# ramanathanlab/molecular_dynamics_neural_operator

Measured on AMD Instinct MI355X. Metric: rolled-out MD frames/sec, higher is better.
Workload: dtype f32

## Files before the change

molecular_dynamics_neural_operator_amd/csrc/moment.hip:

```cpp
#include <type_traits>

#include "kernels.h"
#include "mfma_f32.h"
#include "moment_layout.h"
#include "split_mma.h"

namespace mdno {
namespace {

typedef float f32x4 __attribute__((ext_vector_type(4)));


__global__ __launch_bounds__(256) void w3_moment_kernel(const float* __restrict__ w3, const float* __restrict__ b3, int k,
                                                        float* __restrict__ w3r) {
    const long long id = (long long)blockIdx.x * 256 + threadIdx.x;
    const long long total = (long long)(64 * k + 64) * 64;
    if (id >= total) return;
    const int kl = (int)(id & 31), o = (int)((id >> 5) & 63);
    const long long kappa = (id >> 11) * 32 + kl;
    if (kappa >= (long long)64 * k) {
        w3r[id] = b3[(kappa - (long long)64 * k) * 64 + o];
        return;
    }
    const int i = (int)(kappa / k), c = (int)(kappa - (long long)i * k);
    w3r[id] = w3[((size_t)i * 64 + o) * k + c];
}

__global__ __launch_bounds__(256) void w3_colmax_kernel(const float* __restrict__ w3r, long long ntiles, int* __restrict__ colmax_bits) {
    __shared__ int red[4][64];
    const int o = threadIdx.x & 63, sub = threadIdx.x >> 6;
    float m = 0.f;
    for (long long t = (long long)blockIdx.x * 4 + sub; t < ntiles; t += (long long)gridDim.x * 4) {
        const float4* row = reinterpret_cast<const float4*>(w3r + (t * 64 + o) * 32);
#pragma unroll
        for (int j = 0; j < 8; ++j) {
            const float4 v = row[j];
            const float a = fabsf(v.x), b = fabsf(v.y), c = fabsf(v.z), d = fabsf(v.w);
            m = (a > m || a != a) ? a : m; m = (b > m || b != b) ? b : m;
            m = (c > m || c != c) ? c : m; m = (d > m || d != d) ? d : m;
        }
    }
    red[sub][o] = __builtin_bit_cast(int, m);
    __syncthreads();
    if (sub == 0) {
        int v = red[0][o];
        for (int u = 1; u < 4; ++u) v = red[u][o] > v ? red[u][o] : v;
        atomicMax(colmax_bits + o, v);
    }
}

__global__ __launch_bounds__(256) void w3_planes_f16_kernel(const float* __restrict__ w3r, long long total,
                                                            const int* __restrict__ colmax_bits, _Float16* __restrict__ w3h,
                                                            float* __restrict__ colinv) {
    const long long id = (long long)blockIdx.x * 256 + threadIdx.x;
    if (id < 64) colinv[id] = 1.f / f16_row_scale(__builtin_bit_cast(float, colmax_bits[id]));
    if (id >= total) return;
    const int kl = (int)(id & 31), o = (int)((id >> 5) & 63);
    const long long tile = id >> 11;
    const float v = w3r[id] * f16_row_scale(__builtin_bit_cast(float, colmax_bits[o]));
    const _Float16 h = (_Float16)v;
    w3h[(tile * 2 + 0) * 2048 + o * 32 + kl] = h;
    w3h[(tile * 2 + 1) * 2048 + o * 32 + kl] = (_Float16)(v - (float)h);
}

template <int CH>
__global__ __launch_bounds__(CH) void degree_order_kernel(const int* __restrict__ row_ptr, int num_rows,
                                                          int* __restrict__ order) {
    __shared__ __attribute__((aligned(16))) int key[CH];
    const int base = blockIdx.x * CH, t = threadIdx.x;
    const int cnt = num_rows - base < CH ? num_rows - base : CH;
    int dg = t < cnt ? row_ptr[base + t + 1] - row_ptr[base + t] : 0;
    dg = dg < (1 << 20) ? dg : (1 << 20);
    const int mine = t < cnt ? dg * CH + (CH - 1 - t) : -1;
    key[t] = mine;
    __syncthreads();
    if (t >= cnt) return;
    int rank = 0;
#pragma unroll 4
    for (int u = 0; u < CH; u += 4) {
        const int4 k4 = *reinterpret_cast<const int4*>(&key[u]);
        rank += (k4.x > mine) + (k4.y > mine) + (k4.z > mine) + (k4.w > mine);
    }
    order[base + rank] = t;
}

constexpr int MO_EDGES = 16;
constexpr size_t kMomentCachedBytes = (size_t)64 << 20;
constexpr int MO_HROW = MO_CQ * 2 + 64;
constexpr int MO_XROW = 64 * 2 + 64;
constexpr int MO_HPLANE = MO_EDGES * MO_HROW, MO_XPLANE = MO_EDGES * MO_XROW;
constexpr int MO_LDS = 3 * MO_HPLANE + 3 * MO_XPLANE;

__device__ __forceinline__ int f32_exponent(float p2) { return (int)((__builtin_bit_cast(unsigned, p2) >> 23) & 0xffu) - 127; }

__device__ __forceinline__ float wave_max(float v) {
#pragma unroll
    for (int off = 32; off > 0; off >>= 1) v = fmaxf(v, __shfl_xor(v, off, 64));
    return v;
}

__device__ __forceinline__ void moment_s0(const int* __restrict__ row_ptr, const int* __restrict__ src,
                                          const float* __restrict__ x, float* __restrict__ S, int K, int t, int tl,
                                          float* __restrict__ rowmax_slot, float scale) {
    __shared__ float4 sred[16][16];
    const int tid = threadIdx.x;
    const int beg = row_ptr[t], end = row_ptr[t + 1];
    const int es = tid >> 4, q = tid & 15;
    float4 s0 = make_float4(0.f, 0.f, 0.f, 0.f);
    for (int p = beg + es; p < end; p += 64) {
        int sj[4];
        bool on[4];
#pragma unroll
        for (int u = 0; u < 4; ++u) {
            on[u] = p + 16 * u < end;
            sj[u] = on[u] ? src[p + 16 * u] : 0;
        }
        float4 g[4];
#pragma unroll
        for (int u = 0; u < 4; ++u)
            g[u] = on[u] ? *reinterpret_cast<const float4*>(x + (size_t)sj[u] * 64 + 4 * q) : make_float4(0.f, 0.f, 0.f, 0.f);
#pragma unroll
        for (int u = 0; u < 4; ++u) { s0.x += g[u].x; s0.y += g[u].y; s0.z += g[u].z; s0.w += g[u].w; }
    }
    sred[es][q] = s0;
    __syncthreads();
    float4 s0r = make_float4(0.f, 0.f, 0.f, 0.f);
    if (es == 0) {
        float4 a = make_float4(0.f, 0.f, 0.f, 0.f);
#pragma unroll
        for (int c = 0; c < 16; ++c) { const float4 v = sred[c][q]; a.x += v.x; a.y += v.y; a.z += v.z; a.w += v.w; }
        a.x *= scale; a.y *= scale; a.z *= scale; a.w *= scale;
        s0r = a;
        const int i = 4 * q;
        float* d = S + ((size_t)(tl >> 7) * moment_nkt(K) + (size_t)64 * K / 32 + (i >> 5)) * 4096 + (tl & 127) * 32 + (i & 31);
        *reinterpret_cast<float4*>(d) = a;
    }
    if (rowmax_slot != nullptr && tid < 64) {
        float m = es == 0 ? fmaxf(fmaxf(fabsf(s0r.x), fabsf(s0r.y)), fmaxf(fabsf(s0r.z), fabsf(s0r.w))) : 0.f;
        m = wave_max(m);
        if (tid == 0) *rowmax_slot = m;
    }
}

constexpr int MOMENT_CNT_K1_RERUN = 0;
constexpr int MOMENT_CNT_X_PLAIN = 1;
constexpr int MO_F16_PRE_H_EXP = 5;
constexpr float MO_F16_PRE_H = 32.f, MO_F16_H_LIM = F16_MAX / 32.f, MO_F16_H_MIN = 0.25f / 32.f;

template <bool F16>
__global__ __launch_bounds__(256, 3) void moment_kernel(const float* __restrict__ Hm,
                                                        const int* __restrict__ row_ptr, const int* __restrict__ src,
                                                        const int* __restrict__ order, float* __restrict__ S, int K,
                                                        int row0, int cnt, const float* __restrict__ x, int cache_e,
                                                        float* __restrict__ rowmax, const float* __restrict__ xm,
                                                        int* __restrict__ counters) {
    __shared__ __attribute__((aligned(16))) unsigned char lds[MO_LDS];
    __shared__ float wg_red[12];
    const int nq = (K + MO_CQ - 1) / MO_CQ + 1;
    const int xcd = blockIdx.x & 7, rr = blockIdx.x >> 3;
    const int cq = rr % nq, ti = (rr / nq) * 8 + xcd;
    if (ti >= cnt) return;
    const int tl = order[row0 + ti];
    const int t = row0 + tl;
    const int beg = row_ptr[t], end = row_ptr[t + 1];
    const int tid = threadIdx.x, lane = tid & 63;
    const int wave = __builtin_amdgcn_readfirstlane(tid >> 6);
    const int nkt = K >> 5;
    float xsc = 1.f, hsc = 1.f;
    bool x_plain = false;
    if constexpr (F16) {
        float m = 0.f;
        for (int e = beg + tid; e < end; e += 256) m = fmaxf(m, xm[src[e]]);
        m = wave_max(m);
        if (lane == 0) wg_red[wave] = m;
        __syncthreads();
        m = fmaxf(fmaxf(wg_red[0], wg_red[1]), fmaxf(wg_red[2], wg_red[3]));
        x_plain = !(m >= 0x1p-100f && m < 0x1p100f);
        xsc = x_plain ? 1.f : __builtin_bit_cast(float, __builtin_amdgcn_readfirstlane(__builtin_bit_cast(int, f16_row_scale(m))));
        hsc = x_plain ? 1.f : MO_F16_PRE_H;
        __syncthreads();
        if (cq == 0 && tid == 0) {
            rowmax[(size_t)tl * (nq + 1) + nq] = x_plain ? 0.f : (float)(f32_exponent(xsc) + MO_F16_PRE_H_EXP);
            if (x_plain) atomicAdd(counters + MOMENT_CNT_X_PLAIN, 1);
        }
    }
    if (cq == nq - 1) {
        moment_s0(row_ptr, src, x, S, K, t, tl, rowmax ? rowmax + (size_t)tl * (nq + 1) + cq : nullptr, xsc * hsc);
        return;
    }
    const int er = tid >> 4, cc = tid & 15;
    const int xe = tid >> 4, xs = tid & 15;
    auto h_ptr = [&](int e, int u) {
        const int c = cq * MO_CQ + u * 64 + cc * 4;
        return Hm + ((size_t)(e >> 7) * nkt + (c >> 5)) * 4096 + (e & 127) * 32 + (c & 31);
    };
    float4 rh[4], rx;
    int sidx = 0;
#define MO_NT(DST, P)                                                                               \
    {                                                                                               \
        const f32x4 t_ = __builtin_nontemporal_load(reinterpret_cast<const f32x4*>(P));             \
        DST = make_float4(t_.x, t_.y, t_.z, t_.w);                                                  \
    }
    auto load_stage = [&](int e0) {
        const int e = e0 + er;
        if (e0 + MO_EDGES <= cache_e) {
#pragma unroll
            for (int u = 0; u < 4; ++u) {
                rh[u] = make_float4(0.f, 0.f, 0.f, 0.f);
                if (e < end && cq * MO_CQ + u * 64 < K) rh[u] = *reinterpret_cast<const float4*>(h_ptr(e, u));
            }
        } else {
#pragma unroll
            for (int u = 0; u < 4; ++u) {
                rh[u] = make_float4(0.f, 0.f, 0.f, 0.f);
                if (e < end && cq * MO_CQ + u * 64 < K) MO_NT(rh[u], h_ptr(e, u))
            }
        }
        rx = make_float4(0.f, 0.f, 0.f, 0.f);
        if (e0 + xe < end) rx = *reinterpret_cast<const float4*>(x + (size_t)sidx * 64 + 4 * xs);
    };
    const int gq = lane >> 4, qq = (lane >> 2) & 3, pp = lane & 3;
    const int frow = 8 * (gq >> 1) + qq, fcol = 16 * (gq & 1) + 4 * pp;
    const unsigned char* hb = lds + frow * MO_HROW + (wave * 64 + fcol) * 2;
    const unsigned char* xb = lds + 3 * MO_HPLANE + frow * MO_XROW + fcol * 2;
    auto tr_frag = [&](const unsigned char* p_, int row_bytes) {
        typedef short s16x4 __attribute__((ext_vector_type(4)));
        typedef __attribute__((address_space(3))) s16x4 lds_s16x4;
        const s16x4 lo = __builtin_amdgcn_ds_read_tr16_b64_v4i16((lds_s16x4*)(p_));
        const s16x4 hi = __builtin_amdgcn_ds_read_tr16_b64_v4i16((lds_s16x4*)(p_ + 4 * row_bytes));
        return __builtin_shufflevector(lo, hi, 0, 1, 2, 3, 4, 5, 6, 7);
    };
    f32x16 acc[2][2];
    const int stages = (end - beg + MO_EDGES - 1) / MO_EDGES;
    const bool wave_live = cq * MO_CQ + wave * 64 < K;
    float hmax = 0.f;
    auto max4 = [](const float4 v) { return fmaxf(fmaxf(fabsf(v.x), fabsf(v.y)), fmaxf(fabsf(v.z), fabsf(v.w))); };
    auto pre = [](const float4 v, float sc) { return make_float4(v.x * sc, v.y * sc, v.z * sc, v.w * sc); };
    auto wg_max2 = [&](float a, float b, float& ra, float& rb) {
        a = wave_max(a); b = wave_max(b);
        if (lane == 0) { wg_red[wave] = a; wg_red[4 + wave] = b; }
        __syncthreads();
        ra = fmaxf(fmaxf(wg_red[0], wg_red[1]), fmaxf(wg_red[2], wg_red[3]));
        rb = fmaxf(fmaxf(wg_red[4], wg_red[5]), fmaxf(wg_red[6], wg_red[7]));
    };

    auto run = [&](auto half_tag) {
        constexpr bool HALF = decltype(half_tag)::value;
        auto store_stage = [&]() {
            if constexpr (HALF) {
#pragma unroll
                for (int u = 0; u < 4; ++u) {
                    hmax = fmaxf(hmax, max4(rh[u]));
                    split2_store4(pre(rh[u], hsc), lds + er * MO_HROW + (u * 64 + cc * 4) * 2, MO_HPLANE);
                }
                split2_store4(pre(rx, xsc), lds + 3 * MO_HPLANE + xe * MO_XROW + xs * 8, MO_XPLANE);
            } else if constexpr (F16) {
#pragma unroll
                for (int u = 0; u < 4; ++u)
                    split_store4(pre(rh[u], hsc), lds + er * MO_HROW + (u * 64 + cc * 4) * 2, MO_HPLANE);
                split_store4(pre(rx, xsc), lds + 3 * MO_HPLANE + xe * MO_XROW + xs * 8, MO_XPLANE);
            } else {
#pragma unroll
                for (int u = 0; u < 4; ++u)
                    split_store4(rh[u], lds + er * MO_HROW + (u * 64 + cc * 4) * 2, MO_HPLANE);
                split_store4(rx, lds + 3 * MO_HPLANE + xe * MO_XROW + xs * 8, MO_XPLANE);
            }
        };
#pragma unroll
        for (int i = 0; i < 2; ++i)
#pragma unroll
            for (int j = 0; j < 2; ++j)
#pragma unroll
                for (int e = 0; e < 16; ++e) acc[i][j][e] = 0.f;
        if (stages == 0) return;
        sidx = 0;
        if (beg + xe < end) sidx = src[beg + xe];
        load_stage(beg);
        if (beg + MO_EDGES + xe < end) sidx = src[beg + MO_EDGES + xe];
        store_stage();
        __syncthreads();
        for (int st = 0; st < stages; ++st) {
            const int e_next = beg + (st + 1) * MO_EDGES;
            if (st + 1 < stages) {
                load_stage(e_next);
                if (e_next + MO_EDGES + xe < end) sidx = src[e_next + MO_EDGES + xe];
            }
            __builtin_amdgcn_sched_barrier(0);
            if (wave_live) {
                if constexpr (HALF) {
                    f16x8 a[2][2], b[2];
#pragma unroll
                    for (int ih = 0; ih < 2; ++ih)
#pragma unroll
                        for (int p = 0; p < 2; ++p)
                            a[ih][p] = __builtin_bit_cast(f16x8, tr_frag(xb + p * MO_XPLANE + ih * 64, MO_XROW));
#pragma unroll
                    for (int cb = 0; cb < 2; ++cb) {
#pragma unroll
                        for (int p = 0; p < 2; ++p) b[p] = __builtin_bit_cast(f16x8, tr_frag(hb + p * MO_HPLANE + cb * 64, MO_HROW));
                        mma3_f16(a[0], b, acc[0][cb]);
                        mma3_f16(a[1], b, acc[1][cb]);
                    }
                } else {
                    bf16x8 a[2][3], b[3];
#pragma unroll
                    for (int ih = 0; ih < 2; ++ih)
#pragma unroll
                        for (int p = 0; p < 3; ++p)
                            a[ih][p] = __builtin_bit_cast(bf16x8, tr_frag(xb + p * MO_XPLANE + ih * 64, MO_XROW));
#pragma unroll
                    for (int cb = 0; cb < 2; ++cb) {
#pragma unroll
                        for (int p = 0; p < 3; ++p) b[p] = __builtin_bit_cast(bf16x8, tr_frag(hb + p * MO_HPLANE + cb * 64, MO_HROW));
                        mma6_bf16(a[0], b, acc[0][cb]);
                        mma6_bf16(a[1], b, acc[1][cb]);
                    }
                }
            }
            if (st + 1 < stages) {
                __syncthreads();
                store_stage();
                __syncthreads();
            }
        }
    };
    if constexpr (F16) {
        run(std::true_type{});
        float mh, d;
        wg_max2(hmax, 0.f, mh, d);
        if (stages != 0 && (x_plain || !(mh < MO_F16_H_LIM && mh >= MO_F16_H_MIN))) {
            if (tid == 0) atomicAdd(counters + MOMENT_CNT_K1_RERUN, 1);
            __syncthreads();
            run(std::false_type{});
        }
    } else {
        run(std::false_type{});
    }
#undef MO_NT
    float smax = 0.f;
    if (wave_live) {
        const int l31 = lane & 31, h = lane >> 5;
        float* Sb = S + (size_t)(tl >> 7) * moment_nkt(K) * 4096 + (tl & 127) * 32 + l31;
#pragma unroll
        for (int ih = 0; ih < 2; ++ih)
#pragma unroll
            for (int cb = 0; cb < 2; ++cb) {
                const int c0 = cq * MO_CQ + wave * 64 + cb * 32;
#pragma unroll
                for (int e = 0; e < 16; ++e) {
                    const int i = mfma32_row(e, h, ih * 32);
                    const size_t kt = ((size_t)i * K + c0) >> 5;
                    const float v = acc[ih][cb][e];
                    Sb[kt * 4096] = v;
                    smax = fmaxf(smax, fabsf(v));
                }
            }
    }
    if (rowmax != nullptr) {
        __syncthreads();
        float m, d;
        wg_max2(smax, 0.f, m, d);
        if (tid == 0) rowmax[(size_t)tl * (nq + 1) + cq] = m;
    }
}

constexpr int MF_HLD = MO_CQ + 32, MF_XLD = 64 + 32;

__global__ __launch_bounds__(256) void moment_f32_kernel(const float* __restrict__ Hm, const int* __restrict__ row_ptr,
                                                         const int* __restrict__ src, const int* __restrict__ order,
                                                         float* __restrict__ S, int K, int row0, int cnt,
                                                         const float* __restrict__ x) {
    __shared__ __attribute__((aligned(16))) float hs[MO_EDGES * MF_HLD];
    __shared__ __attribute__((aligned(16))) float xs_[MO_EDGES * MF_XLD];
    const int nq = (K + MO_CQ - 1) / MO_CQ + 1;
    const int xcd = blockIdx.x & 7, rr = blockIdx.x >> 3;
    const int cq = rr % nq, ti = (rr / nq) * 8 + xcd;
    if (ti >= cnt) return;
    const int tl = order[row0 + ti];
    const int t = row0 + tl;
    if (cq == nq - 1) {
        moment_s0(row_ptr, src, x, S, K, t, tl, nullptr, 1.f);
        return;
    }
    const int beg = row_ptr[t], end = row_ptr[t + 1];
    const int tid = threadIdx.x, lane = tid & 63;
    const int wave = __builtin_amdgcn_readfirstlane(tid >> 6);
    const int er = tid >> 4, cc = tid & 15;
    const int l31 = lane & 31, h = lane >> 5;
    const bool wave_live = cq * MO_CQ + wave * 64 < K;
    f32x16 acc[2][2];
#pragma unroll
    for (int i = 0; i < 2; ++i)
#pragma unroll
        for (int j = 0; j < 2; ++j)
#pragma unroll
            for (int e = 0; e < 16; ++e) acc[i][j][e] = 0.f;
    for (int e0 = beg; e0 < end; e0 += MO_EDGES) {
        const int e = e0 + er;
        float4 rh[4], rx = make_float4(0.f, 0.f, 0.f, 0.f);
#pragma unroll
        for (int u = 0; u < 4; ++u) {
            rh[u] = make_float4(0.f, 0.f, 0.f, 0.f);
            const int c = cq * MO_CQ + u * 64 + cc * 4;
            if (e < end && c < K)
                rh[u] = *reinterpret_cast<const float4*>(Hm + ((size_t)(e >> 7) * (K >> 5) + (c >> 5)) * 4096 + (e & 127) * 32 + (c & 31));
        }
        if (e < end) rx = *reinterpret_cast<const float4*>(x + (size_t)src[e] * 64 + 4 * cc);
        __syncthreads();
#pragma unroll
        for (int u = 0; u < 4; ++u) *reinterpret_cast<float4*>(&hs[er * MF_HLD + u * 64 + cc * 4]) = rh[u];
        *reinterpret_cast<float4*>(&xs_[er * MF_XLD + cc * 4]) = rx;
        __syncthreads();
        if (wave_live) {
#pragma unroll
            for (int ks = 0; ks < MO_EDGES / 2; ++ks) {
                const float a0 = xs_[(2 * ks + h) * MF_XLD + l31], a1 = xs_[(2 * ks + h) * MF_XLD + 32 + l31];
                const float b0 = hs[(2 * ks + h) * MF_HLD + wave * 64 + l31], b1 = hs[(2 * ks + h) * MF_HLD + wave * 64 + 32 + l31];
                acc[0][0] = __builtin_amdgcn_mfma_f32_32x32x2f32(a0, b0, acc[0][0], 0, 0, 0);
                acc[0][1] = __builtin_amdgcn_mfma_f32_32x32x2f32(a0, b1, acc[0][1], 0, 0, 0);
                acc[1][0] = __builtin_amdgcn_mfma_f32_32x32x2f32(a1, b0, acc[1][0], 0, 0, 0);
                acc[1][1] = __builtin_amdgcn_mfma_f32_32x32x2f32(a1, b1, acc[1][1], 0, 0, 0);
            }
        }
    }
    if (!wave_live) return;
    float* Sb = S + (size_t)(tl >> 7) * moment_nkt(K) * 4096 + (tl & 127) * 32 + l31;
#pragma unroll
    for (int ih = 0; ih < 2; ++ih)
#pragma unroll
        for (int cb = 0; cb < 2; ++cb) {
            const int c0 = cq * MO_CQ + wave * 64 + cb * 32;
#pragma unroll
            for (int e = 0; e < 16; ++e) {
                const int i = mfma32_row(e, h, ih * 32);
                const size_t kt = ((size_t)i * K + c0) >> 5;
                Sb[kt * 4096] = acc[ih][cb][e];
            }
        }
}

constexpr int PJ_SLICES = 128;
constexpr int PJ_B_PLANE = 64 * 64;

template <int PJ_ROWS>
__global__ __launch_bounds__(PJ_ROWS * 2) void project_kernel(const float* __restrict__ S, const float* __restrict__ w3r,
                                                         float* __restrict__ part, int K, int cnt, int row0,
                                                         long long part_stride) {
    constexpr int PJ_A_PLANE = PJ_ROWS * 64, PJ_B_BASE = 3 * PJ_A_PLANE, NT = PJ_ROWS / 128;
    constexpr int RQ = PJ_ROWS / 4;
    __shared__ __attribute__((aligned(16))) unsigned char lds[3 * PJ_A_PLANE + 3 * PJ_B_PLANE];
    const int ngrp = gridDim.x / PJ_SLICES;
    const int xcd = blockIdx.x & 7, rr = blockIdx.x >> 3;
    const int rg = rr % ngrp, slice = (rr / ngrp) * 8 + xcd;
    const int tid = threadIdx.x, lane = tid & 63;
    const int wave = __builtin_amdgcn_readfirstlane(tid >> 6);
    const int l31 = lane & 31, h = lane >> 5;
    const int srow = tid >> 3, scol = (tid & 7) * 4;
    const int nkt = (int)moment_nkt(K), per = (nkt - 2) / PJ_SLICES;
    const int kt0 = slice * per, nk = per + (slice == PJ_SLICES - 1 ? 2 : 0);
    const int first = rg * PJ_ROWS;
    const int rows_here = cnt - first < PJ_ROWS ? cnt - first : PJ_ROWS;
    const int live = (rows_here + 31) >> 5;
    auto a_ptr = [&](int r) {
        return S + ((size_t)(NT * rg + (r >> 7)) * nkt + kt0) * 4096 + (r & 127) * 32 + scol;
    };
    auto a_row = [&](int r) { return r < rows_here ? r : rows_here - 1; };
    const float* A0 = a_ptr(a_row(srow));
    const float* A1 = a_ptr(a_row(srow + RQ));
    const float* A2 = a_ptr(a_row(srow + 2 * RQ));
    const float* A3 = a_ptr(a_row(srow + 3 * RQ));
    const float* Bg = w3r + (size_t)kt0 * 2048 + srow * 32 + scol;
    struct Tile { float4 a0, a1, a2, a3, b0, b1; };
    auto load = [&](Tile& r, int kt) {
        r.a0 = *reinterpret_cast<const float4*>(A0 + (size_t)kt * 4096);
        r.a1 = *reinterpret_cast<const float4*>(A1 + (size_t)kt * 4096);
        r.a2 = *reinterpret_cast<const float4*>(A2 + (size_t)kt * 4096);
        r.a3 = *reinterpret_cast<const float4*>(A3 + (size_t)kt * 4096);
        r.b0 = *reinterpret_cast<const float4*>(Bg + (size_t)kt * 2048);
        if (RQ < 64) r.b1 = *reinterpret_cast<const float4*>(Bg + (size_t)kt * 2048 + RQ * 32);
    };
    auto st_off = [&](int row) { return row * 64 + ((((tid & 7) >> 1) ^ ((row >> 2) & 3)) << 4) + (tid & 1) * 8; };
    unsigned char* a_st0 = lds + st_off(srow);
    unsigned char* a_st1 = lds + st_off(srow + RQ);
    unsigned char* a_st2 = lds + st_off(srow + 2 * RQ);
    unsigned char* a_st3 = lds + st_off(srow + 3 * RQ);
    unsigned char* b_st0 = lds + PJ_B_BASE + st_off(srow);
    unsigned char* b_st1 = lds + PJ_B_BASE + st_off(srow + RQ);
    auto store = [&](const Tile& r) {
        split_store4(r.a0, a_st0, PJ_A_PLANE);
        split_store4(r.a1, a_st1, PJ_A_PLANE);
        split_store4(r.a2, a_st2, PJ_A_PLANE);
        split_store4(r.a3, a_st3, PJ_A_PLANE);
        split_store4(r.b0, b_st0, PJ_B_PLANE);
        if (RQ < 64) split_store4(r.b1, b_st1, PJ_B_PLANE);
    };
    f32x16 acc0, acc1;
#pragma unroll
    for (int e = 0; e < 16; ++e) { acc0[e] = 0.f; acc1[e] = 0.f; }
    const int arow = wave * 32 + l31, brow0 = l31, brow1 = 32 + l31;
    const int a_sw = (arow >> 2) & 3, b_sw0 = (brow0 >> 2) & 3, b_sw1 = (brow1 >> 2) & 3;
    const unsigned char* a_rd = lds + arow * 64;
    const unsigned char* b_rd0 = lds + PJ_B_BASE + brow0 * 64;
    const unsigned char* b_rd1 = lds + PJ_B_BASE + brow1 * 64;
#define PJ_MMA_TILE()                                                                                    \
    _Pragma("unroll") for (int st = 0; st < 2; ++st) {                                                   \
        bf16x8 a[3], b0[3], b1[3];                                                                       \
        _Pragma("unroll") for (int p = 0; p < 3; ++p) {                                                  \
            a[p] = *reinterpret_cast<const bf16x8*>(a_rd + p * PJ_A_PLANE + (((2 * st + h) ^ a_sw) << 4));   \
            b0[p] = *reinterpret_cast<const bf16x8*>(b_rd0 + p * PJ_B_PLANE + (((2 * st + h) ^ b_sw0) << 4)); \
            b1[p] = *reinterpret_cast<const bf16x8*>(b_rd1 + p * PJ_B_PLANE + (((2 * st + h) ^ b_sw1) << 4)); \
        }                                                                                                \
        mma6_bf16(a, b0, acc0); mma6_bf16(a, b1, acc1);                                                  \
    }
    const bool rows_live = wave < live;
    Tile P, Q;
    const int last = nk - 1;
    load(P, 0);
    load(Q, 1);
    store(P);
    __syncthreads();
    for (int kt = 0;; kt += 2) {
        load(P, min(kt + 2, last));
        __builtin_amdgcn_sched_barrier(0);
        if (rows_live) { PJ_MMA_TILE() }
        __syncthreads();
        store(Q);
        __syncthreads();
        load(Q, min(kt + 3, last));
        __builtin_amdgcn_sched_barrier(0);
        if (rows_live) { PJ_MMA_TILE() }
        if (kt + 2 >= nk) break;
        __syncthreads();
        store(P);
        __syncthreads();
    }
#undef PJ_MMA_TILE
    float* Po = part + (size_t)slice * part_stride;
#pragma unroll
    for (int e = 0; e < 16; ++e) {
        const int m = mfma32_row(e, h, first + wave * 32);
        if (m < cnt) {
            Po[(size_t)(row0 + m) * 64 + l31] = acc0[e];
            Po[(size_t)(row0 + m) * 64 + 32 + l31] = acc1[e];
        }
    }
}

__global__ __launch_bounds__(512) void project_f16_kernel(const float* __restrict__ S, const unsigned short* __restrict__ w3h_bits,
                                                          float* __restrict__ part, int K, int cnt, int row0,
                                                          long long part_stride, const float* __restrict__ rowmax, int nq,
                                                          const float* __restrict__ colinv) {
    const _Float16* __restrict__ w3h = reinterpret_cast<const _Float16*>(w3h_bits);
    constexpr int PJ_ROWS = 256, PJ_A_PLANE = PJ_ROWS * 64, PJ_B_BASE = 2 * PJ_A_PLANE, NT = 2, RQ = 64;
    __shared__ __attribute__((aligned(16))) unsigned char lds[2 * PJ_A_PLANE + 2 * PJ_B_PLANE];
    __shared__ int rowexp[PJ_ROWS];
    const int ngrp = gridDim.x / PJ_SLICES;
    const int xcd = blockIdx.x & 7, rr = blockIdx.x >> 3;
    const int rg = rr % ngrp, slice = (rr / ngrp) * 8 + xcd;
    const int tid = threadIdx.x, lane = tid & 63;
    const int wave = __builtin_amdgcn_readfirstlane(tid >> 6);
    const int l31 = lane & 31, h = lane >> 5;
    const int srow = tid >> 3, scol = (tid & 7) * 4;
    const int nkt = (int)moment_nkt(K), per = (nkt - 2) / PJ_SLICES;
    const int kt0 = slice * per, nk = per + (slice == PJ_SLICES - 1 ? 2 : 0);
    const int first = rg * PJ_ROWS;
    const int rows_here = cnt - first < PJ_ROWS ? cnt - first : PJ_ROWS;
    const int live = (rows_here + 31) >> 5;
    auto a_row = [&](int r) { return r < rows_here ? r : rows_here - 1; };
    auto a_ptr = [&](int r) {
        return S + ((size_t)(NT * rg + (r >> 7)) * nkt + kt0) * 4096 + (r & 127) * 32 + scol;
    };
    auto row_scale = [&](int r) {
        const float* m = rowmax + (size_t)(first + r) * (nq + 1);
        float v = 0.f;
        for (int q = 0; q < nq; ++q) v = fmaxf(v, m[q]);
        return f16_row_scale(v);
    };
    auto row_exp = [&](int r) { return (int)rowmax[(size_t)(first + r) * (nq + 1) + nq]; };
    const int r0_ = a_row(srow), r1_ = a_row(srow + RQ), r2_ = a_row(srow + 2 * RQ), r3_ = a_row(srow + 3 * RQ);
    const float* A0 = a_ptr(r0_);
    const float* A1 = a_ptr(r1_);
    const float* A2 = a_ptr(r2_);
    const float* A3 = a_ptr(r3_);
    const float sc0 = row_scale(r0_), sc1 = row_scale(r1_), sc2 = row_scale(r2_), sc3 = row_scale(r3_);
    if ((tid & 7) == 0) {
        rowexp[srow] = f32_exponent(sc0) + row_exp(r0_); rowexp[srow + RQ] = f32_exponent(sc1) + row_exp(r1_);
        rowexp[srow + 2 * RQ] = f32_exponent(sc2) + row_exp(r2_); rowexp[srow + 3 * RQ] = f32_exponent(sc3) + row_exp(r3_);
    }
    const int bp = tid >> 8, bo = (tid >> 2) & 63, bc = tid & 3;
    const _Float16* Bg = w3h + ((size_t)kt0 * 2 + bp) * 2048 + bo * 32 + bc * 8;
    struct Tile { float4 a0, a1, a2, a3; uint4 b; };
    auto load = [&](Tile& r, int kt) {
        r.a0 = *reinterpret_cast<const float4*>(A0 + (size_t)kt * 4096);
        r.a1 = *reinterpret_cast<const float4*>(A1 + (size_t)kt * 4096);
        r.a2 = *reinterpret_cast<const float4*>(A2 + (size_t)kt * 4096);
        r.a3 = *reinterpret_cast<const float4*>(A3 + (size_t)kt * 4096);
        r.b = *reinterpret_cast<const uint4*>(Bg + (size_t)kt * 4096);
    };
    auto st_off = [&](int row) { return row * 64 + ((((tid & 7) >> 1) ^ ((row >> 2) & 3)) << 4) + (tid & 1) * 8; };
    unsigned char* a_st0 = lds + st_off(srow);
    unsigned char* a_st1 = lds + st_off(srow + RQ);
    unsigned char* a_st2 = lds + st_off(srow + 2 * RQ);
    unsigned char* a_st3 = lds + st_off(srow + 3 * RQ);
    unsigned char* b_st = lds + PJ_B_BASE + bp * PJ_B_PLANE + bo * 64 + ((bc ^ ((bo >> 2) & 3)) << 4);
    auto scaled = [](const float4 v, float sc) { return make_float4(v.x * sc, v.y * sc, v.z * sc, v.w * sc); };
    auto store = [&](const Tile& r) {
        split2_store4(scaled(r.a0, sc0), a_st0, PJ_A_PLANE);
        split2_store4(scaled(r.a1, sc1), a_st1, PJ_A_PLANE);
        split2_store4(scaled(r.a2, sc2), a_st2, PJ_A_PLANE);
        split2_store4(scaled(r.a3, sc3), a_st3, PJ_A_PLANE);
        *reinterpret_cast<uint4*>(b_st) = r.b;
    };
    f32x16 acc0, acc1;
#pragma unroll
    for (int e = 0; e < 16; ++e) { acc0[e] = 0.f; acc1[e] = 0.f; }
    const int arow = wave * 32 + l31, brow0 = l31, brow1 = 32 + l31;
    const int a_sw = (arow >> 2) & 3, b_sw0 = (brow0 >> 2) & 3, b_sw1 = (brow1 >> 2) & 3;
    const unsigned char* a_rd = lds + arow * 64;
    const unsigned char* b_rd0 = lds + PJ_B_BASE + brow0 * 64;
    const unsigned char* b_rd1 = lds + PJ_B_BASE + brow1 * 64;
#define PJ_MMA_TILE()                                                                                    \
    _Pragma("unroll") for (int st = 0; st < 2; ++st) {                                                   \
        f16x8 a[2], b0[2], b1[2];                                                                        \
        _Pragma("unroll") for (int p = 0; p < 2; ++p) {                                                  \
            a[p] = *reinterpret_cast<const f16x8*>(a_rd + p * PJ_A_PLANE + (((2 * st + h) ^ a_sw) << 4));    \
            b0[p] = *reinterpret_cast<const f16x8*>(b_rd0 + p * PJ_B_PLANE + (((2 * st + h) ^ b_sw0) << 4)); \
            b1[p] = *reinterpret_cast<const f16x8*>(b_rd1 + p * PJ_B_PLANE + (((2 * st + h) ^ b_sw1) << 4)); \
        }                                                                                                \
        mma3_f16(a, b0, acc0); mma3_f16(a, b1, acc1);                                                    \
    }
    const bool rows_live = wave < live;
    Tile P, Q;
    const int last = nk - 1;
    load(P, 0);
    load(Q, 1);
    store(P);
    __syncthreads();
    for (int kt = 0;; kt += 2) {
        load(P, min(kt + 2, last));
        __builtin_amdgcn_sched_barrier(0);
        if (rows_live) { PJ_MMA_TILE() }
        __syncthreads();
        store(Q);
        __syncthreads();
        load(Q, min(kt + 3, last));
        __builtin_amdgcn_sched_barrier(0);
        if (rows_live) { PJ_MMA_TILE() }
        if (kt + 2 >= nk) break;
        __syncthreads();
        store(P);
        __syncthreads();
    }
#undef PJ_MMA_TILE
    const int ec0 = f32_exponent(colinv[l31]), ec1 = f32_exponent(colinv[32 + l31]);
    float* Po = part + (size_t)slice * part_stride;
#pragma unroll
    for (int e = 0; e < 16; ++e) {
        const int ml = mfma32_row(e, h, wave * 32), m = first + ml;
        if (m < cnt) {
            const int er = rowexp[ml];
            Po[(size_t)(row0 + m) * 64 + l31] = ldexpf(acc0[e], ec0 - er);
            Po[(size_t)(row0 + m) * 64 + 32 + l31] = ldexpf(acc1[e], ec1 - er);
        }
    }
}

__global__ __launch_bounds__(256) void project_f32_kernel(const float* __restrict__ S, const float* __restrict__ w3r,
                                                          float* __restrict__ part, int K, int cnt, int row0,
                                                          long long part_stride) {
    using namespace f32mma;
    __shared__ __attribute__((aligned(16))) float As[128 * LD];
    __shared__ __attribute__((aligned(16))) float Bs[64 * LD];
    const int ngrp = gridDim.x / PJ_SLICES;
    const int xcd = blockIdx.x & 7, rr = blockIdx.x >> 3;
    const int rg = rr % ngrp, slice = (rr / ngrp) * 8 + xcd;
    const int tid = threadIdx.x, lane = tid & 63;
    const int wave = __builtin_amdgcn_readfirstlane(tid >> 6);
    const int l31 = lane & 31, h = lane >> 5;
    const int srow = tid >> 3, scol = (tid & 7) * 4;
    const int nkt = (int)moment_nkt(K), per = (nkt - 2) / PJ_SLICES;
    const int kt0 = slice * per, nk = per + (slice == PJ_SLICES - 1 ? 2 : 0);
    const int first = rg * 128;
    const float* Ag = S + ((size_t)rg * nkt + kt0) * 4096 + srow * 32 + scol;
    const float* Bg = w3r + (size_t)kt0 * 2048 + srow * 32 + scol;
    f32x16 acc0, acc1;
#pragma unroll
    for (int e = 0; e < 16; ++e) { acc0[e] = 0.f; acc1[e] = 0.f; }
    for (int kt = 0; kt < nk; ++kt) {
        float4 a[4], b[2];
#pragma unroll
        for (int j = 0; j < 4; ++j) a[j] = *reinterpret_cast<const float4*>(Ag + (size_t)kt * 4096 + j * 32 * 32);
#pragma unroll
        for (int j = 0; j < 2; ++j) b[j] = *reinterpret_cast<const float4*>(Bg + (size_t)kt * 2048 + j * 32 * 32);
        __syncthreads();
#pragma unroll
        for (int j = 0; j < 4; ++j) *reinterpret_cast<float4*>(&As[(srow + 32 * j) * LD + scol]) = a[j];
#pragma unroll
        for (int j = 0; j < 2; ++j) *reinterpret_cast<float4*>(&Bs[(srow + 32 * j) * LD + scol]) = b[j];
        __syncthreads();
        mma_32x64(acc0, acc1, &As[(wave * 32 + l31) * LD + 4 * h], &Bs[l31 * LD + 4 * h]);
    }
    float* Po = part + (size_t)slice * part_stride;
#pragma unroll
    for (int e = 0; e < 16; ++e) {
        const int m = mfma32_row(e, h, first + wave * 32);
        if (m < cnt) {
            Po[(size_t)(row0 + m) * 64 + l31] = acc0[e];
            Po[(size_t)(row0 + m) * 64 + 32 + l31] = acc1[e];
        }
    }
}

constexpr int FN_CHAINS = 32;

__global__ __launch_bounds__(FN_CHAINS * 16) void finish_kernel(const float* __restrict__ part, long long part_stride,
                                                                const int* __restrict__ row_ptr, const float* __restrict__ x,
                                                                const float* __restrict__ root, const float* __restrict__ bias,
                                                                float* __restrict__ y, int row0, int aggr, int relu,
                                                                float* __restrict__ xm_out) {
    constexpr int CPT = 64 / FN_CHAINS;
    __shared__ float4 red[FN_CHAINS][16];
    __shared__ float4 red2[FN_CHAINS][16];
    const int tid = threadIdx.x, es = tid >> 4, q = tid & 15;
    const int t = row0 + blockIdx.x;
    const int deg = row_ptr[t + 1] - row_ptr[t];
    float4 rootv[CPT], biasv = make_float4(0.f, 0.f, 0.f, 0.f);
    float xin[CPT];
#pragma unroll
    for (int i = 0; i < CPT; ++i) {
        rootv[i] = make_float4(0.f, 0.f, 0.f, 0.f);
        xin[i] = 0.f;
        if (root != nullptr) {
            xin[i] = x[(size_t)t * 64 + CPT * es + i];
            rootv[i] = *reinterpret_cast<const float4*>(root + (CPT * es + i) * 64 + 4 * q);
        }
    }
    if (bias != nullptr && es == 0) biasv = *reinterpret_cast<const float4*>(bias + 4 * q);
    float4 z = make_float4(0.f, 0.f, 0.f, 0.f);
    {
        float4 v[PJ_SLICES / FN_CHAINS];
#pragma unroll
        for (int u = 0; u < PJ_SLICES / FN_CHAINS; ++u)
            v[u] = *reinterpret_cast<const float4*>(part + (size_t)(es + u * FN_CHAINS) * part_stride + (size_t)t * 64 + 4 * q);
#pragma unroll
        for (int u = 0; u < PJ_SLICES / FN_CHAINS; ++u) { z.x += v[u].x; z.y += v[u].y; z.z += v[u].z; z.w += v[u].w; }
    }
    float4 racc = make_float4(0.f, 0.f, 0.f, 0.f);
#pragma unroll
    for (int i = 0; i < CPT; ++i) {
        racc.x = fmaf(xin[i], rootv[i].x, racc.x); racc.y = fmaf(xin[i], rootv[i].y, racc.y);
        racc.z = fmaf(xin[i], rootv[i].z, racc.z); racc.w = fmaf(xin[i], rootv[i].w, racc.w);
    }
    red[es][q] = z;
    red2[es][q] = racc;
    __syncthreads();
    if (es == 0) {
        float4 s = make_float4(0.f, 0.f, 0.f, 0.f), rs = make_float4(0.f, 0.f, 0.f, 0.f);
#pragma unroll
        for (int c = 0; c < FN_CHAINS; ++c) {
            const float4 a = red[c][q], b = red2[c][q];
            s.x += a.x; s.y += a.y; s.z += a.z; s.w += a.w;
            rs.x += b.x; rs.y += b.y; rs.z += b.z; rs.w += b.w;
        }
        if (aggr == MDNO_AGGR_MEAN) {
            const float inv = (float)(deg > 1 ? deg : 1);
            s.x /= inv; s.y /= inv; s.z /= inv; s.w /= inv;
        }
        if (root != nullptr) { s.x += rs.x; s.y += rs.y; s.z += rs.z; s.w += rs.w; }
        if (bias != nullptr) { s.x += biasv.x; s.y += biasv.y; s.z += biasv.z; s.w += biasv.w; }
        if (relu) { s.x = relu_f(s.x); s.y = relu_f(s.y); s.z = relu_f(s.z); s.w = relu_f(s.w); }
        *reinterpret_cast<float4*>(y + (size_t)t * 64 + 4 * q) = s;
        if (xm_out != nullptr) {
            float m = fmaxf(fmaxf(fabsf(s.x), fabsf(s.y)), fmaxf(fabsf(s.z), fabsf(s.w)));
#pragma unroll
            for (int off = 8; off > 0; off >>= 1) m = fmaxf(m, __shfl_xor(m, off, 64));
            if (q == 0) xm_out[t] = m;
        }
    }
}

__global__ __launch_bounds__(256) void row_absmax_kernel(const float* __restrict__ x, int num_rows, float* __restrict__ xm) {
    const int r = blockIdx.x * 16 + (threadIdx.x >> 4), q = threadIdx.x & 15;
    float m = 0.f;
    if (r < num_rows) {
        const float4 v = *reinterpret_cast<const float4*>(x + (size_t)r * 64 + 4 * q);
        m = fmaxf(fmaxf(fabsf(v.x), fabsf(v.y)), fmaxf(fabsf(v.z), fabsf(v.w)));
    }
#pragma unroll
    for (int off = 8; off > 0; off >>= 1) m = fmaxf(m, __shfl_xor(m, off, 64));
    if (q == 0 && r < num_rows) xm[r] = m;
}


}


bool moment_supported(int width, int ker_width) { return width == 64 && ker_width >= 128 && ker_width % 128 == 0; }
static int moment_nq(int ker_width) { return (ker_width + MO_CQ - 1) / MO_CQ + 1; }
static size_t s_chunk_floats(int num_rows, int ker_width) { return (size_t)(moment_chunk_rows(num_rows) / 128) * moment_nkt(ker_width) * 4096; }

static MomentWs moment_carve_impl(Carver& cv, int num_rows, int ker_width) {
    MomentWs f{};
    f.w3r = cv.take<float>((size_t)(64 * ker_width + 64) * 64);
    f.s = cv.take<float>(s_chunk_floats(num_rows, ker_width));
    f.part = cv.take<float>((size_t)PJ_SLICES * num_rows * 64);
    f.part_stride = (long long)num_rows * 64;
    f.order = cv.take<int>((size_t)num_rows);
    f.w3h = cv.take<_Float16>((size_t)(64 * ker_width + 64) * 64 * 2);
    f.colinv = cv.take<float>(64);
    f.colmax_bits = cv.take<int>(64);
    f.rowmax = cv.take<float>((size_t)(moment_chunk_rows(num_rows) + 256) * (moment_nq(ker_width) + 1));
    f.xm[0] = cv.take<float>((size_t)num_rows);
    f.xm[1] = cv.take<float>((size_t)num_rows);
    f.counters = cv.take<int>(64);
    return f;
}

size_t moment_workspace_bytes(int num_rows, int ker_width) {
    Carver cv(nullptr);
    (void)moment_carve_impl(cv, num_rows, ker_width);
    return cv.used();
}

MomentWs moment_carve(void* ws, int num_rows, int ker_width) {
    Carver cv(ws);
    return moment_carve_impl(cv, num_rows, ker_width);
}

int moment_prepare_weights(const float* w3, const float* b3, int ker_width, const MomentWs& f, hipStream_t s, int gemm_mode) {
    const long long total = (long long)(64 * ker_width + 64) * 64;
    hipLaunchKernelGGL(w3_moment_kernel, dim3((unsigned)((total + 255) / 256)), dim3(256), 0, s, w3, b3, ker_width, f.w3r);
    if (gemm_mode == MDNO_GEMM_SPLIT_F16) {
        MDNO_HIP(hipMemsetAsync(f.colmax_bits, 0, 64 * sizeof(int), s));
        hipLaunchKernelGGL(w3_colmax_kernel, dim3(256), dim3(256), 0, s, (const float*)f.w3r, total / 2048, f.colmax_bits);
        hipLaunchKernelGGL(w3_planes_f16_kernel, dim3((unsigned)((total + 255) / 256)), dim3(256), 0, s, (const float*)f.w3r, total,
                           (const int*)f.colmax_bits, f.w3h, f.colinv);
    }
    return check_launch("w3_moment_kernel");
}

int moment_prepare_graph(const int* row_ptr, int num_rows, const MomentWs& f, hipStream_t s) {
    TimedSection ts(KID_GRAPH, s);
    hipLaunchKernelGGL(degree_order_kernel<kMomentChunkRows>, dim3((num_rows + kMomentChunkRows - 1) / kMomentChunkRows),
                       dim3(kMomentChunkRows), 0, s, row_ptr, num_rows, f.order);
    return check_launch("degree_order_kernel");
}

int moment_row_absmax(const float* x, int num_rows, const MomentWs& f, hipStream_t s) {
    hipLaunchKernelGGL(row_absmax_kernel, dim3((num_rows + 15) / 16), dim3(256), 0, s, x, num_rows, f.xm[0]);
    return check_launch("row_absmax_kernel");
}

int moment_s_chunk(const float* x, const float* h2, const int* row_ptr, const int* src, int ker_width, int r0, int cnt,
                   const MomentWs& f, hipStream_t s, bool exact_f32) {
    const dim3 grid((unsigned)(((cnt + 7) / 8) * 8 * moment_nq(ker_width)));
    const int cache_e = (int)(kMomentCachedBytes / ((size_t)ker_width * sizeof(float))) & ~127;
    if (exact_f32)
        hipLaunchKernelGGL(moment_f32_kernel, grid, dim3(256), 0, s, h2, row_ptr, src, (const int*)f.order, f.s, ker_width, r0,
                           cnt, x);
    else
        hipLaunchKernelGGL(moment_kernel<false>, grid, dim3(256), 0, s, h2, row_ptr, src, (const int*)f.order, f.s, ker_width,
                           r0, cnt, x, cache_e, (float*)nullptr, (const float*)nullptr, (int*)nullptr);
    return check_launch("moment_s_chunk");
}

int moment_conv(const float* x, const float* h2, const int* row_ptr, const int* src, int num_rows, int ker_width,
                const float* root, const float* bias, int aggr, int relu, float* y, const MomentWs& f, hipStream_t s,
                int gemm_mode, int application) {
    MDNO_REQUIRE(moment_supported(64, ker_width), MDNO_EUNSUPPORTED, "moment conv: ker_width=%d (x128)", ker_width);
    const bool exact_f32 = gemm_mode == MDNO_GEMM_F32, f16 = gemm_mode == MDNO_GEMM_SPLIT_F16;
    const int nq = moment_nq(ker_width);
    const float* xm_in = f.xm[application & 1];
    float* xm_out = f16 ? f.xm[(application + 1) & 1] : nullptr;
    size_t cached_bytes = kMomentCachedBytes;
#ifdef MDNO_EXP_CACHE_ENV
    if (const char* v = getenv("MDNO_EXP_CACHE_MIB")) cached_bytes = (size_t)atoi(v) << 20;
#endif
    const int cache_e = (int)(cached_bytes / ((size_t)ker_width * sizeof(float))) & ~127;
    for (int r0 = 0; r0 < num_rows; r0 += kMomentChunkRows) {
        const int cnt = num_rows - r0 < kMomentChunkRows ? num_rows - r0 : kMomentChunkRows;
        {
            TimedSection ts(KID_NNCONV, s);
            const dim3 grid((unsigned)(((cnt + 7) / 8) * 8 * nq));
            if (exact_f32)
                hipLaunchKernelGGL(moment_f32_kernel, grid, dim3(256), 0, s, h2, row_ptr, src, (const int*)f.order, f.s,
                                   ker_width, r0, cnt, x);
            else if (f16)
                hipLaunchKernelGGL(moment_kernel<true>, grid, dim3(256), 0, s, h2, row_ptr, src, (const int*)f.order, f.s, ker_width,
                                   r0, cnt, x, cache_e, f.rowmax, xm_in, f.counters);
            else
                hipLaunchKernelGGL(moment_kernel<false>, grid, dim3(256), 0, s, h2, row_ptr, src, (const int*)f.order, f.s, ker_width,
                                   r0, cnt, x, cache_e, (float*)nullptr, (const float*)nullptr, (int*)nullptr);
        }
        {
            TimedSection ts(KID_FACT_Y, s);
            if (exact_f32)
                hipLaunchKernelGGL(project_f32_kernel, dim3(((cnt + 127) / 128) * PJ_SLICES), dim3(256), 0, s, (const float*)f.s,
                                   (const float*)f.w3r, f.part, ker_width, cnt, r0, f.part_stride);
            else if (f16)
                hipLaunchKernelGGL(project_f16_kernel, dim3(((cnt + 255) / 256) * PJ_SLICES), dim3(512), 0, s, (const float*)f.s,
                                   reinterpret_cast<const unsigned short*>(f.w3h), f.part, ker_width, cnt, r0, f.part_stride,
                                   (const float*)f.rowmax, nq, (const float*)f.colinv);
            else
                hipLaunchKernelGGL(project_kernel<256>, dim3(((cnt + 255) / 256) * PJ_SLICES), dim3(512), 0, s, (const float*)f.s,
                                   (const float*)f.w3r, f.part, ker_width, cnt, r0, f.part_stride);
        }
        {
            TimedSection ts(KID_NNCONV_COMBINE, s);
            hipLaunchKernelGGL(finish_kernel, dim3(cnt), dim3(FN_CHAINS * 16), 0, s, (const float*)f.part, f.part_stride,
                               row_ptr, x, root, bias, y, r0, aggr, relu, xm_out);
        }
    }
    return check_launch("moment_conv");
}

}
```

Baseline: 592.3.

## Restructure f16 projection into per-chain blocks that pre-reduce four slices

The f16 projection kernel now gives each block one reduction chain: four of the K slices over 64 rows, split across a 2x2 wave grid. Each block loads two k-tiles per stage into double-buffered LDS and folds the scaled accumulators into a per-chain sum in registers. The finish kernel then reads one partial per chain instead of summing four slice partials. This cuts partial-buffer writes and reads and reduces finish work, at the cost of longer serial K loops per block, half the waves idle in MMA, and a different grid shape that changes occupancy.

```diff
diff --git a/molecular_dynamics_neural_operator_amd/csrc/moment.hip b/molecular_dynamics_neural_operator_amd/csrc/moment.hip
--- a/molecular_dynamics_neural_operator_amd/csrc/moment.hip
+++ b/molecular_dynamics_neural_operator_amd/csrc/moment.hip
@@ -440,6 +440,7 @@
 }
 
 constexpr int PJ_SLICES = 128;
+constexpr int FN_CHAINS = 32;
 constexpr int PJ_B_PLANE = 64 * 64;
 
 template <int PJ_ROWS>
@@ -546,122 +547,128 @@
     }
 }
 
-__global__ __launch_bounds__(512) void project_f16_kernel(const float* __restrict__ S, const unsigned short* __restrict__ w3h_bits,
-                                                          float* __restrict__ part, int K, int cnt, int row0,
+constexpr int PJ_CHAIN_ROWS = 64;
+constexpr int PJ_F16_SETS = 2;
+static_assert(PJ_SLICES == 4 * FN_CHAINS && PJ_F16_SETS % 2 == 0, "project_f16_kernel: four slices per chain, two LDS buffers");
+__global__ __launch_bounds__(512) void project_f16_kernel(const float* S, const unsigned short* w3h_bits,
+                                                          float* part, int K, int cnt, int row0,
                                                           long long part_stride, const float* __restrict__ rowmax, int nq,
                                                           const float* __restrict__ colinv) {
-    const _Float16* __restrict__ w3h = reinterpret_cast<const _Float16*>(w3h_bits);
-    constexpr int PJ_ROWS = 256, PJ_A_PLANE = PJ_ROWS * 64, PJ_B_BASE = 2 * PJ_A_PLANE, NT = 2, RQ = 64;
-    __shared__ __attribute__((aligned(16))) unsigned char lds[2 * PJ_A_PLANE + 2 * PJ_B_PLANE];
-    __shared__ int rowexp[PJ_ROWS];
-    const int ngrp = gridDim.x / PJ_SLICES;
+    const _Float16* w3h = reinterpret_cast<const _Float16*>(w3h_bits);
+    constexpr int ROWS = PJ_CHAIN_ROWS, A_PLANE = ROWS * 64, B_BASE = 2 * A_PLANE, TILE = 2 * A_PLANE + 2 * PJ_B_PLANE;
+    constexpr int STAGE = 2 * TILE, NSET = PJ_F16_SETS;
+    __shared__ __attribute__((aligned(16))) unsigned char lds[2 * STAGE];
+    __shared__ int rowexp[ROWS];
+    const int ngrp = gridDim.x / FN_CHAINS;
     const int xcd = blockIdx.x & 7, rr = blockIdx.x >> 3;
-    const int rg = rr % ngrp, slice = (rr / ngrp) * 8 + xcd;
+    const int rg = rr % ngrp, es = (rr / ngrp) * 8 + xcd;
     const int tid = threadIdx.x, lane = tid & 63;
     const int wave = __builtin_amdgcn_readfirstlane(tid >> 6);
     const int l31 = lane & 31, h = lane >> 5;
     const int srow = tid >> 3, scol = (tid & 7) * 4;
-    const int nkt = (int)moment_nkt(K), per = (nkt - 2) / PJ_SLICES;
-    const int kt0 = slice * per, nk = per + (slice == PJ_SLICES - 1 ? 2 : 0);
-    const int first = rg * PJ_ROWS;
-    const int rows_here = cnt - first < PJ_ROWS ? cnt - first : PJ_ROWS;
+    const int nkt = (int)moment_nkt(K), per = (nkt - 2) / PJ_SLICES, hs = per >> 1;
+    const int last = 4 * hs - 1 + (es == FN_CHAINS - 1 ? 1 : 0);
+    int ld_i = 0, ld_kt = es * per;
+    auto next_stage = [&]() {
+        const bool jump = ld_i + 1 == hs || ld_i + 1 == 2 * hs || ld_i + 1 == 3 * hs;
+        const int step = ld_i < last ? 2 + (jump ? (FN_CHAINS - 1) * per : 0) : 0;
+        ld_kt += step;
+        ld_i += ld_i < last ? 1 : 0;
+    };
+    const int first = rg * ROWS;
+    const int rows_here = cnt - first < ROWS ? cnt - first : ROWS;
     const int live = (rows_here + 31) >> 5;
-    auto a_row = [&](int r) { return r < rows_here ? r : rows_here - 1; };
-    auto a_ptr = [&](int r) {
-        return S + ((size_t)(NT * rg + (r >> 7)) * nkt + kt0) * 4096 + (r & 127) * 32 + scol;
-    };
-    auto row_scale = [&](int r) {
-        const float* m = rowmax + (size_t)(first + r) * (nq + 1);
-        float v = 0.f;
-        for (int q = 0; q < nq; ++q) v = fmaxf(v, m[q]);
-        return f16_row_scale(v);
-    };
-    auto row_exp = [&](int r) { return (int)rowmax[(size_t)(first + r) * (nq + 1) + nq]; };
-    const int r0_ = a_row(srow), r1_ = a_row(srow + RQ), r2_ = a_row(srow + 2 * RQ), r3_ = a_row(srow + 3 * RQ);
-    const float* A0 = a_ptr(r0_);
-    const float* A1 = a_ptr(r1_);
-    const float* A2 = a_ptr(r2_);
-    const float* A3 = a_ptr(r3_);
-    const float sc0 = row_scale(r0_), sc1 = row_scale(r1_), sc2 = row_scale(r2_), sc3 = row_scale(r3_);
-    if ((tid & 7) == 0) {
-        rowexp[srow] = f32_exponent(sc0) + row_exp(r0_); rowexp[srow + RQ] = f32_exponent(sc1) + row_exp(r1_);
-        rowexp[srow + 2 * RQ] = f32_exponent(sc2) + row_exp(r2_); rowexp[srow + 3 * RQ] = f32_exponent(sc3) + row_exp(r3_);
-    }
+    const int rc = first + (srow < rows_here ? srow : rows_here - 1);
+    const float* Ag = S + (size_t)(rc >> 7) * nkt * 4096 + (rc & 127) * 32 + scol;
+    const float* rm = rowmax + (size_t)rc * (nq + 1);
+    float rmax = 0.f;
+    for (int q = 0; q < nq; ++q) rmax = fmaxf(rmax, rm[q]);
+    const float sc = f16_row_scale(rmax);
+    if ((tid & 7) == 0) rowexp[srow] = f32_exponent(sc) + (int)rm[nq];
     const int bp = tid >> 8, bo = (tid >> 2) & 63, bc = tid & 3;
-    const _Float16* Bg = w3h + ((size_t)kt0 * 2 + bp) * 2048 + bo * 32 + bc * 8;
-    struct Tile { float4 a0, a1, a2, a3; uint4 b; };
-    auto load = [&](Tile& r, int kt) {
-        r.a0 = *reinterpret_cast<const float4*>(A0 + (size_t)kt * 4096);
-        r.a1 = *reinterpret_cast<const float4*>(A1 + (size_t)kt * 4096);
-        r.a2 = *reinterpret_cast<const float4*>(A2 + (size_t)kt * 4096);
-        r.a3 = *reinterpret_cast<const float4*>(A3 + (size_t)kt * 4096);
-        r.b = *reinterpret_cast<const uint4*>(Bg + (size_t)kt * 4096);
-    };
-    auto st_off = [&](int row) { return row * 64 + ((((tid & 7) >> 1) ^ ((row >> 2) & 3)) << 4) + (tid & 1) * 8; };
-    unsigned char* a_st0 = lds + st_off(srow);
-    unsigned char* a_st1 = lds + st_off(srow + RQ);
-    unsigned char* a_st2 = lds + st_off(srow + 2 * RQ);
-    unsigned char* a_st3 = lds + st_off(srow + 3 * RQ);
-    unsigned char* b_st = lds + PJ_B_BASE + bp * PJ_B_PLANE + bo * 64 + ((bc ^ ((bo >> 2) & 3)) << 4);
-    auto scaled = [](const float4 v, float sc) { return make_float4(v.x * sc, v.y * sc, v.z * sc, v.w * sc); };
-    auto store = [&](const Tile& r) {
-        split2_store4(scaled(r.a0, sc0), a_st0, PJ_A_PLANE);
-        split2_store4(scaled(r.a1, sc1), a_st1, PJ_A_PLANE);
-        split2_store4(scaled(r.a2, sc2), a_st2, PJ_A_PLANE);
-        split2_store4(scaled(r.a3, sc3), a_st3, PJ_A_PLANE);
-        *reinterpret_cast<uint4*>(b_st) = r.b;
-    };
-    f32x16 acc0, acc1;
-#pragma unroll
-    for (int e = 0; e < 16; ++e) { acc0[e] = 0.f; acc1[e] = 0.f; }
-    const int arow = wave * 32 + l31, brow0 = l31, brow1 = 32 + l31;
-    const int a_sw = (arow >> 2) & 3, b_sw0 = (brow0 >> 2) & 3, b_sw1 = (brow1 >> 2) & 3;
-    const unsigned char* a_rd = lds + arow * 64;
-    const unsigned char* b_rd0 = lds + PJ_B_BASE + brow0 * 64;
-    const unsigned char* b_rd1 = lds + PJ_B_BASE + brow1 * 64;
-#define PJ_MMA_TILE()                                                                                    \
-    _Pragma("unroll") for (int st = 0; st < 2; ++st) {                                                   \
-        f16x8 a[2], b0[2], b1[2];                                                                        \
-        _Pragma("unroll") for (int p = 0; p < 2; ++p) {                                                  \
-            a[p] = *reinterpret_cast<const f16x8*>(a_rd + p * PJ_A_PLANE + (((2 * st + h) ^ a_sw) << 4));    \
-            b0[p] = *reinterpret_cast<const f16x8*>(b_rd0 + p * PJ_B_PLANE + (((2 * st + h) ^ b_sw0) << 4)); \
-            b1[p] = *reinterpret_cast<const f16x8*>(b_rd1 + p * PJ_B_PLANE + (((2 * st + h) ^ b_sw1) << 4)); \
-        }                                                                                                \
-        mma3_f16(a, b0, acc0); mma3_f16(a, b1, acc1);                                                    \
-    }
-    const bool rows_live = wave < live;
-    Tile P, Q;
-    const int last = nk - 1;
-    load(P, 0);
-    load(Q, 1);
-    store(P);
-    __syncthreads();
-    for (int kt = 0;; kt += 2) {
-        load(P, min(kt + 2, last));
-        __builtin_amdgcn_sched_barrier(0);
-        if (rows_live) { PJ_MMA_TILE() }
-        __syncthreads();
-        store(Q);
-        __syncthreads();
-        load(Q, min(kt + 3, last));
-        __builtin_amdgcn_sched_barrier(0);
-        if (rows_live) { PJ_MMA_TILE() }
-        if (kt + 2 >= nk) break;
-        __syncthreads();
-        store(P);
-        __syncthreads();
-    }
-#undef PJ_MMA_TILE
-    const int ec0 = f32_exponent(colinv[l31]), ec1 = f32_exponent(colinv[32 + l31]);
-    float* Po = part + (size_t)slice * part_stride;
+    const _Float16* Bg = w3h + (size_t)bp * 2048 + bo * 32 + bc * 8;
+    struct Stage { float4 a0, a1; uint4 b0, b1; };
+    auto load = [&](Stage& r) {
+        const size_t kt = (size_t)ld_kt;
+        next_stage();
+        r.a0 = *reinterpret_cast<const float4*>(Ag + kt * 4096);
+        r.a1 = *reinterpret_cast<const float4*>(Ag + (kt + 1) * 4096);
+        r.b0 = *reinterpret_cast<const uint4*>(Bg + kt * 4096);
+        r.b1 = *reinterpret_cast<const uint4*>(Bg + (kt + 1) * 4096);
+        asm volatile("" ::: "memory");
+    };
+    const int a_st = srow * 64 + ((((tid & 7) >> 1) ^ ((srow >> 2) & 3)) << 4) + (tid & 1) * 8;
+    const int b_st = B_BASE + bp * PJ_B_PLANE + bo * 64 + ((bc ^ ((bo >> 2) & 3)) << 4);
+    auto scaled = [](const float4 v, float s_) { return make_float4(v.x * s_, v.y * s_, v.z * s_, v.w * s_); };
+    auto store = [&](const Stage& r, int buf) {
+        unsigned char* base = lds + buf * STAGE;
+        float sc_ = sc;
+        asm volatile("" : "+v"(sc_));
+        split2_store4(scaled(r.a0, sc_), base + a_st, A_PLANE);
+        split2_store4(scaled(r.a1, sc_), base + TILE + a_st, A_PLANE);
+        *reinterpret_cast<uint4*>(base + b_st) = r.b0;
+        *reinterpret_cast<uint4*>(base + TILE + b_st) = r.b1;
+    };
+    f32x16 acc, chain;
+#pragma unroll
+    for (int e = 0; e < 16; ++e) { acc[e] = 0.f; chain[e] = 0.f; }
+    const int rb = (wave >> 1) & 1, cb = wave & 1;
+    const int arow = rb * 32 + l31, brow = cb * 32 + l31;
+    const int a_sw = (arow >> 2) & 3, b_sw = (brow >> 2) & 3;
+    const int a_rd = arow * 64, b_rd = B_BASE + brow * 64;
+    const bool mma_wave = wave < 4 && rb < live;
+    const int ec = f32_exponent(colinv[cb * 32 + l31]);
+    auto mma_tile = [&](const unsigned char* base) {
+#pragma unroll
+        for (int st = 0; st < 2; ++st) {
+            f16x8 a[2], b[2];
+#pragma unroll
+            for (int p = 0; p < 2; ++p) {
+                a[p] = *reinterpret_cast<const f16x8*>(base + a_rd + p * A_PLANE + (((2 * st + h) ^ a_sw) << 4));
+                b[p] = *reinterpret_cast<const f16x8*>(base + b_rd + p * PJ_B_PLANE + (((2 * st + h) ^ b_sw) << 4));
+            }
+            mma3_f16(a, b, acc);
+        }
+    };
+    Stage R[NSET];
+    auto multiply = [&](int i, int buf) {
+        if (!mma_wave) return;
+        mma_tile(lds + buf * STAGE);
+        mma_tile(lds + buf * STAGE + TILE);
+        if (i + 1 == hs || i + 1 == 2 * hs || i + 1 == 3 * hs || i == last) {
+#pragma unroll
+            for (int e = 0; e < 16; ++e) {
+                chain[e] = chain[e] + ldexpf(acc[e], ec - rowexp[mfma32_row(e, h, rb * 32)]);
+                acc[e] = 0.f;
+            }
+        }
+    };
+    int i0 = -NSET;
+    for (; i0 + NSET <= last + 1; i0 += NSET) {
+#pragma unroll
+        for (int j = 0; j < NSET; ++j) {
+            load(R[j]);
+            __builtin_amdgcn_sched_barrier(0);
+            if (i0 >= 0) multiply(i0 + j, j & 1);
+            if (i0 >= 0 || j == NSET - 1) {
+                store(R[(j + 1) % NSET], (j + 1) & 1);
+                __syncthreads();
+            }
+        }
+    }
+#pragma unroll
+    for (int j = 0; j < NSET - 1; ++j)
+        if (i0 + j <= last) {
+            multiply(i0 + j, j & 1);
+            store(R[j + 1], (j + 1) & 1);
+            __syncthreads();
+        }
+    if (!mma_wave) return;
+    float* Po = part + (size_t)es * part_stride + cb * 32 + l31;
 #pragma unroll
     for (int e = 0; e < 16; ++e) {
-        const int ml = mfma32_row(e, h, wave * 32), m = first + ml;
-        if (m < cnt) {
-            const int er = rowexp[ml];
-            Po[(size_t)(row0 + m) * 64 + l31] = ldexpf(acc0[e], ec0 - er);
-            Po[(size_t)(row0 + m) * 64 + 32 + l31] = ldexpf(acc1[e], ec1 - er);
-        }
+        const int m = mfma32_row(e, h, first + rb * 32);
+        if (m < cnt) Po[(size_t)(row0 + m) * 64] = chain[e];
     }
 }
 
@@ -711,8 +718,7 @@
     }
 }
 
-constexpr int FN_CHAINS = 32;
-
+template <int PPC>
 __global__ __launch_bounds__(FN_CHAINS * 16) void finish_kernel(const float* __restrict__ part, long long part_stride,
                                                                 const int* __restrict__ row_ptr, const float* __restrict__ x,
                                                                 const float* __restrict__ root, const float* __restrict__ bias,
@@ -736,14 +742,17 @@
         }
     }
     if (bias != nullptr && es == 0) biasv = *reinterpret_cast<const float4*>(bias + 4 * q);
+    static_assert(PPC == 1 || PPC == PJ_SLICES / FN_CHAINS, "finish_kernel: chain partials or slice partials");
     float4 z = make_float4(0.f, 0.f, 0.f, 0.f);
-    {
-        float4 v[PJ_SLICES / FN_CHAINS];
-#pragma unroll
-        for (int u = 0; u < PJ_SLICES / FN_CHAINS; ++u)
+    if (PPC == 1) {
+        z = *reinterpret_cast<const float4*>(part + (size_t)es * part_stride + (size_t)t * 64 + 4 * q);
+    } else {
+        float4 v[PPC];
+#pragma unroll
+        for (int u = 0; u < PPC; ++u)
             v[u] = *reinterpret_cast<const float4*>(part + (size_t)(es + u * FN_CHAINS) * part_stride + (size_t)t * 64 + 4 * q);
 #pragma unroll
-        for (int u = 0; u < PJ_SLICES / FN_CHAINS; ++u) { z.x += v[u].x; z.y += v[u].y; z.z += v[u].z; z.w += v[u].w; }
+        for (int u = 0; u < PPC; ++u) { z.x += v[u].x; z.y += v[u].y; z.z += v[u].z; z.w += v[u].w; }
     }
     float4 racc = make_float4(0.f, 0.f, 0.f, 0.f);
 #pragma unroll
@@ -898,7 +907,7 @@
                 hipLaunchKernelGGL(project_f32_kernel, dim3(((cnt + 127) / 128) * PJ_SLICES), dim3(256), 0, s, (const float*)f.s,
                                    (const float*)f.w3r, f.part, ker_width, cnt, r0, f.part_stride);
             else if (f16)
-                hipLaunchKernelGGL(project_f16_kernel, dim3(((cnt + 255) / 256) * PJ_SLICES), dim3(512), 0, s, (const float*)f.s,
+                hipLaunchKernelGGL(project_f16_kernel, dim3(((cnt + PJ_CHAIN_ROWS - 1) / PJ_CHAIN_ROWS) * FN_CHAINS), dim3(512), 0, s, (const float*)f.s,
                                    reinterpret_cast<const unsigned short*>(f.w3h), f.part, ker_width, cnt, r0, f.part_stride,
                                    (const float*)f.rowmax, nq, (const float*)f.colinv);
             else
@@ -907,8 +916,12 @@
         }
         {
             TimedSection ts(KID_NNCONV_COMBINE, s);
-            hipLaunchKernelGGL(finish_kernel, dim3(cnt), dim3(FN_CHAINS * 16), 0, s, (const float*)f.part, f.part_stride,
-                               row_ptr, x, root, bias, y, r0, aggr, relu, xm_out);
+            if (f16)
+                hipLaunchKernelGGL(finish_kernel<1>, dim3(cnt), dim3(FN_CHAINS * 16), 0, s, (const float*)f.part, f.part_stride,
+                                   row_ptr, x, root, bias, y, r0, aggr, relu, xm_out);
+            else
+                hipLaunchKernelGGL(finish_kernel<PJ_SLICES / FN_CHAINS>, dim3(cnt), dim3(FN_CHAINS * 16), 0, s, (const float*)f.part,
+                                   f.part_stride, row_ptr, x, root, bias, y, r0, aggr, relu, xm_out);
         }
     }
     return check_launch("moment_conv");
```

Result: faster. 603.5 (median of 6 runs) (+1.9%).
